# Amelie-Schreiber/ShapeMol

Measured on AMD Instinct MI355X. Metric: molecules/sec (1000-step DDPM sample, batch 256), higher is better.
Workload: dtype f32 (matrix operands split exactly into 3 x bf16 pieces = 24 bits, six piece products, fp32 accumulate); 1 GPU; BASELINE configs[1]: batch 256 MOSES-prior molecules (9-27 atoms) per GPU, 1000-step chain, fp32 results, k=8, synthetic shapes + hash-filled weights; besides the 5 warm-up steps an untimed 200-step chain runs first to reach the loaded clocks; batch_per_gpu=256, atoms_per_gpu=5541, total_atoms=5541, noise=device Philox, trajectories=kept in HBM, launch=hipGraph replay, parallelism=dp1 (whole batches per rank), ranks_seen=1

## Files before the change

shapemol_amd/csrc/shapemol_hip.hip:

```cpp
#include "../../include/shapemol_hip.h"
#include "sm_device.h"
#include "sm_edge.h"
#include "sm_edge_bf16.h"
#include "sm_edge16.h"
#include "sm_node.h"
#include "sm_node16.h"
#include "sm_edge_stream.h"
#include "sm_misc.h"
#include "sm_cfg.h"
#include "sm_guide_groups.h"
#include "sm_mesh.h"
#include <hip/hip_ext.h>

#include <algorithm>
#include <cmath>
#include <cstdio>
#include <cstring>
#include <map>
#include <string>
#include <type_traits>
#include <vector>

#include "sm_pack.h"
#include "sm_devmem.h"
// ... 82 lines not shown
    int num_cu = 256;
    CloudSet cs; MeshSet ms; DevList mem_cs, mem_ms;
    int2 *wg_table = nullptr; int64_t wg_table_cap = 0; DevList mem_wg;
    shapemol_sd_ctx *field_sd = nullptr; double field_lr = 0.0; int field_step = 0;
    float4 *m_within = nullptr; int *m_out = nullptr, *m_cnt = nullptr; int64_t m_cap = 0, m_cnt_cap = 0; DevList mem_mesh;
    int64_t m_flag_groups = 0;
    double cfg_w = 0.0, cfg_p = 0.0; int cfg_type = 0, cfg_has_bounds = 0; float cfg_lo[3] = {}, cfg_hi[3] = {};
    float *cfg_tr_pos_u = nullptr, *cfg_tr_v_u = nullptr;
    float *pred_pos_u = nullptr, *pred_v_u = nullptr;
    float *shape_zero = nullptr;
    float *cfg_stat = nullptr; double *cfg_part = nullptr; unsigned *cfg_hist = nullptr;
    CfgGroupSet cgs;
    int *cfg_mol_grp = nullptr; int2 *cfg_blk_tab = nullptr; double *cfg_gpart = nullptr; int64_t cfg_tab_stride = 0;
    int first_step = 0;
    int *pin_off = nullptr, *pin_atom = nullptr, *pin_nbr = nullptr; int64_t n_pins = 0; int pin_steps = 0, pin_k = 0; DevList mem_pins;
    bool prof_on = false;
    std::vector<ProfRec> prof;
    hipEvent_t cur_e0 = nullptr, cur_e1 = nullptr;
    hipGraphExec_t gexec = nullptr, gexec_u = nullptr;
    int64_t n_captures = 0;
    int64_t launch_rec[8] = {}, graph_rec[8] = {};
    int64_t node_rec[8] = {};
    int64_t x2h_out_rec[4] = {};
    struct GraphKey { int64_t N = 0, B = 0; Guide guide = Guide::None; int fold = 0, gfuse = 0;
                      int cfg = 0 ; double cfgv[9] = {};
                      int cfg_groups = 0;
                      uint64_t field_gen = 0; double field_lr = 0.0; int field_step = 0;
                      bool operator==(const GraphKey &o) const {
                          if (!(N == o.N && B == o.B && guide == o.guide && fold == o.fold && gfuse == o.gfuse && cfg == o.cfg &&
                                cfg_groups == o.cfg_groups && field_gen == o.field_gen && field_lr == o.field_lr &&
                                field_step == o.field_step)) return false;
                          for (int i = 0; i < 9; ++i) if (cfgv[i] != o.cfgv[i]) return false;
                          return true;
                      } } gkey{};
    hipStream_t gstream = nullptr; bool gstream_set = false;
    void drop_graphs() {
        if (!gexec && !gexec_u) return;
        if (!gstream_set || hipStreamSynchronize(gstream) != hipSuccess) hipDeviceSynchronize();
        if (gexec) { hipGraphExecDestroy(gexec); gexec = nullptr; }
        if (gexec_u) { hipGraphExecDestroy(gexec_u); gexec_u = nullptr; }
    }
    const float *P(size_t off) const { return d_img + off; }
};

namespace {

// ... 71 lines not shown
    if (N <= c->capN && B <= c->capB) return 0;
    HIPCHK(hipSetDevice(c->device));
    HIPCHK(hipDeviceSynchronize());
    c->drop_graphs();
    const int64_t capN = std::max<int64_t>(N, c->capN), capB = std::max<int64_t>(B, c->capB);
    c->ws.release();
    c->capN = c->capB = 0; c->lastN = c->lastB = 0; c->last_h = c->last_x = nullptr;
    if (workspace_alloc(c, capN, capB)) { c->ws.release(); return 1; }
    c->capN = capN; c->capB = capB;
    return 0;
}

}

#include "sm_guide_host.h"

namespace {

constexpr int kVnFoldBytes = kVnFoldCap * 3 * 4 + 32 * 8;

template <int H>
lg::In launch_in(const shapemol_ctx *c, int n_atoms) {
    constexpr bool chain16_fits = Chain16Lds<H>::BYTES <= 2 * EdgeImage16<H, H / 16>::TOTAL * 4;
    return {c->opt, {kVnFoldCap, kStreamTPR, CHAIN_COLS, kGraphCap, kLin6Chunk, chain16_fits}, c->KP, c->num_cu, H, n_atoms};
}

#define ATTR(bytes, ...) HIPCHK(hipFuncSetAttribute((const void *)__VA_ARGS__, hipFuncAttributeMaxDynamicSharedMemorySize, (int)(bytes)))
template <int H, int K>
int set_edge_attr_k() {
    constexpr int NT = H / 16;
    constexpr int vn_tail = vn_red_doubles(12, H / 8) * 8 + 12 * 96 * 4;
    constexpr int fold = K <= 16 ? kVnFoldBytes : 0;
    constexpr int x16 = 2 * EdgeImage16<H, NT>::TOTAL * 4 + fold, h16 = (EdgeImage16<H, NT>::TOTAL + EdgeImage16<H, 1>::TOTAL) * 4 + vn_tail;
    ATTR(x16, edge16_kernel<H, K, false>); ATTR(x16, edge16_kernel<H, K, false, true>);
    ATTR(x16, edge16_loop_kernel<H, K, false>); ATTR(x16, edge16_loop_kernel<H, K, false, true>);
    ATTR(h16, edge16_kernel<H, K, true>); ATTR(h16, edge16_kernel<H, K, true, true>);
    ATTR(h16, edge16_loop_kernel<H, K, true>); ATTR(h16, edge16_loop_kernel<H, K, true, true>);
    ATTR((StreamMap<H, false>::O_TAIL * 4 + kVnFoldBytes), edge_stream_kernel<H, K, false>);
    ATTR((StreamMap<H, true>::O_TAIL * 4 + (NT + kStreamProducers) * 64 * 2 * 8), edge_stream_kernel<H, K, true>);
    if constexpr (K <= 16) {
        constexpr int xph = EdgePhaseImage<H, NT>::TOTAL * 4, hph = (EdgePhaseImage<H, NT>::TOTAL + EdgePhaseImage<H, 1>::TOTAL) * 4 + vn_tail;
        ATTR(x16, x2h_chain16_kernel<H, K>); ATTR(x16, x2h_chain16_kernel<H, K, true>);
        ATTR((EdgeBlob<H, false>::TOTAL * 4), edge_attention_kernel<H, K, false>); ATTR((EdgeBlob<H, true>::TOTAL * 4), edge_attention_kernel<H, K, true>);
        ATTR(xph, edge_fused_kernel<H, K, false, false>); ATTR(xph, edge_fused_kernel<H, K, false, true>);
        ATTR(hph, edge_fused_kernel<H, K, true, false>); ATTR(hph, edge_fused_kernel<H, K, true, true>);
    }
    return 0;
// ... 321 lines not shown
        HIPCHK(c->mem_tab.alloc(&c->q_tab, rows * 5 * H * sizeof(float) + rows * (sizeof(int64_t) + sizeof(int)) + ((size_t)T + 1) * sizeof(int)));
        c->pre_tab = c->q_tab + rows * H;
        c->tab_v = reinterpret_cast<int64_t *>(c->pre_tab + rows * 4 * H);
        c->tab_mol_of = reinterpret_cast<int *>(c->tab_v + rows); c->tab_t_mol = c->tab_mol_of + rows; c->tab_flag = c->tab_t_mol + T;
    }
    c->tab_key = 0;
    LAUNCH("prep", SMK(prologue_tab_index_kernel, dim3((unsigned)((rows + 255) / 256)), dim3(256), 0, s, c->tab_v, c->tab_mol_of, c->tab_t_mol, c->tab_flag, T, C));
    const NodePrologueArgs pa = prologue_args<H>(c, c->tab_v, c->tab_mol_of, c->tab_t_mol, nullptr, c->etab, c->q_tab, c->pre_tab, (int)rows);
    if (launch_prologue<H>(c, s, pa, c->tab_flag)) return 1;
    c->tab_key = prologue_tab_key(c);
    return 0;
}

template <int H>
int run_score(shapemol_ctx *c, hipStream_t s, const ShapePrep &sp, const float *x_in, const int64_t *v_in, int64_t N, int64_t B,
              bool sampling, int t_first, float *out_pos, float *out_h, float *out_v, bool reuse_graph = false) {
    const shapemol_config &g = c->cfg;
    const int L = g.num_layers, hd = g.n_heads, C = g.num_classes, D = g.time_emb_dim, KP = c->KP;
    const int n = (int)N;
    AtomEmbArgs ae{c->P(c->dm.embw), c->P(c->dm.embb), v_in, c->mol_of, c->ttab, c->t_mol, sampling ? c->steps : nullptr,
                   c->steps + 1, c->bn_acc, c->h_a, n, H, C, D, t_first, L * kVnReplicas * 2 * hd + L};
    const int nlay = c->opt.stop_layer >= 0 ? std::min(c->opt.stop_layer, L) : L;
    const lg::In gi = launch_in<H>(c, n);
    const lg::StepForms sf = lg::step_forms(gi, sampling, c->n_pins > 0);
    if (sf.fused_prologue && c->opt.prologue_tab) {
        if (c->tab_key != prologue_tab_key(c)) return fail("run_score: the prologue tables are not built for this precision mode");
        PrologueTabArgs ta{c->etab, c->q_tab, c->pre_tab, c->tab_flag, v_in, c->mol_of, c->t_mol, ae.step_ptr, ae.step_cur, c->bn_acc,
                           sp.add0, c->h_a, c->q_x, c->pre0, c->status + ST_RANGE, n, C, g.num_timesteps, t_first, ae.bn_acc_len};
        LAUNCH("node_prologue", SMK(node_prologue_tab_kernel<H>, dim3((unsigned)((N * 16 + kProTabThreads - 1) / kProTabThreads)), dim3(kProTabThreads), 0, s, ta));
    } else if (sf.fused_prologue) {
        NodePrologueArgs pa = prologue_args<H>(c, v_in, c->mol_of, c->t_mol, sp.add0, c->h_a, c->q_x, c->pre0, n);
        pa.step_ptr = ae.step_ptr; pa.step_cur = ae.step_cur; pa.bn_acc = c->bn_acc; pa.bn_acc_len = ae.bn_acc_len; pa.t_first = t_first;
        if (nlay == 0) pa.n_lin_tiles = 0;
        pa.stamps = c->kstamp_sel == 5 ? c->kstamps : nullptr;
        if (launch_prologue<H>(c, s, pa)) return 1;
    } else {
        LAUNCH("embed", SMK(atom_embed_kernel, dim3((N * H + 255) / 256), dim3(256), 0, s, ae));
    }
    int64_t (&rec)[8] = c->launch_rec;
    std::fill(rec, rec + 8, 0);
    std::fill(c->node_rec, c->node_rec + 8, 0);
    std::fill(c->x2h_out_rec, c->x2h_out_rec + 4, 0);
    rec[0] = sampling; rec[1] = sf.graph_fused; rec[7] = c->num_cu;
    if (sf.stream && nlay > 0) { const lg::StreamGeom g = lg::stream_geom(gi); rec[5] = g.chunk; rec[6] = g.grid; }
    if (reuse_graph) {
    } else if (sf.graph_fused) {
        GraphArgs ga{x_in, c->mol_span, n, g.knn, KP, c->nbr, c->P(c->dm.ew.w1), c->P(c->dm.ew.b1), c->P(c->dm.ew.g), c->P(c->dm.ew.be),
                     c->P(c->dm.ew.w2), c->P(c->dm.ew.b2), c->ew, c->status + ST_SPAN, c->kstamp_sel == 4 ? c->kstamps : nullptr};
        const int apb = kGraphWaves * (KP >= 16 ? 1 : 16 / KP);
        DISPATCH_KP("graph", graph_kernel, (), dim3((n + apb - 1) / apb), dim3(kGraphWaves * 64), 0, s, ga);
    } else LAUNCH("knn", SMK(knn_kernel, dim3((N + 3) / 4), dim3(256), 0, s, x_in, c->mol_of, c->mol_off, n, g.knn, KP, c->nbr));
    if (sampling && c->n_pins > 0 && !reuse_graph)
        LAUNCH("knn", SMK(knn_pin_kernel, dim3(32), dim3(256), 0, s, c->pin_off, c->pin_steps, c->pin_atom, c->pin_nbr, c->pin_k, KP, c->steps + 1, n, c->nbr));
    EdgeWeightArgs ea{x_in, c->nbr, c->P(c->dm.ew.w1), c->P(c->dm.ew.b1), c->P(c->dm.ew.g), c->P(c->dm.ew.be),
                      c->P(c->dm.ew.w2), c->P(c->dm.ew.b2), c->ew, n * KP, KP};
    if (!sf.graph_fused && !reuse_graph) {
        const int tiles = (n * KP + 15) / 16;
        LAUNCH("edge_weight", SMK(edge_weight_kernel<H>, dim3((tiles + 3) / 4), dim3(256), 0, s, ea));
    }
    const float *cur_x = x_in;
    float *cur_h = c->h_a;
    constexpr int NT = H / 16;
    bool v_done = false;
    if (nlay > 0 && !sf.fused_prologue) {
        const DevLayer &D0 = c->dm.layer[0];
        if (launch_linear<H>(c, s, "node_pre", cur_h, c->P(D0.pre_x2h), c->P(D0.pre6_x2h), c->P(D0.pre16_x2h), sp.add0, 4 * H, c->pre0, 4 * H, 4 * NT, n,
                             c->kstamp_sel == 0 ? c->kstamps : nullptr)) return 1;
        if (launch_mlp2<H, 1>(c, s, "node_q", D0.q_x2h, cur_h, nullptr, NODE_LN_RELU, nullptr, c->q_x, H, H, n)) return 1;
    }
    double *stat_acc = c->bn_acc;
    if (c->bn_eval) {
        if (!c->bn_run) return fail("bn_eval = 1 needs the running statistics (shapemol_set_bn_running)");
        if (c->opt.vn_fuse == 1) return fail("bn_eval = 1 is not available with vn_fuse = 1 (coordinate update behind a grid barrier)");
// ... 319 lines not shown
            const double v[9] = {c->cfg_w, c->cfg_p, (double)c->cfg_has_bounds, c->cfg_lo[0], c->cfg_lo[1], c->cfg_lo[2], c->cfg_hi[0], c->cfg_hi[1], c->cfg_hi[2]};
            std::copy(v, v + 9, key.cfgv);
        }
        auto capture = [&](int n_steps, hipGraphExec_t *exec) -> int {
            hipGraph_t graph = nullptr;
            HIPCHK(hipStreamBeginCapture(s, hipStreamCaptureModeThreadLocal));
            int rc = 0;
            for (int i = 0; i < n_steps && !rc; ++i) rc = one_step();
            const hipError_t ce = hipStreamEndCapture(s, &graph);
            if (rc) { if (graph) hipGraphDestroy(graph); return 1; }
            if (ce != hipSuccess) return fail(std::string("hipStreamEndCapture: ") + hipGetErrorString(ce));
            const hipError_t ie = hipGraphInstantiate(exec, graph, nullptr, nullptr, 0);
            hipGraphDestroy(graph);
            if (ie != hipSuccess) { *exec = nullptr; return fail(std::string("hipGraphInstantiate: ") + hipGetErrorString(ie)); }
            ++c->n_captures;
            hipGraphUpload(*exec, s);
            return 0;
        };
        if (!c->gexec || !(key == c->gkey)) {
            c->drop_graphs();
            if (capture(1, &c->gexec)) return 1;
            c->gkey = key;
            std::copy(c->launch_rec, c->launch_rec + 8, c->graph_rec);
        }
        if (!c->gexec_u && capture(kGraphUnroll, &c->gexec_u)) return 1;
        int st = 0;
        c->gstream = s; c->gstream_set = true;
        std::copy(c->graph_rec, c->graph_rec + 8, c->launch_rec);
        for (; st + kGraphUnroll <= num_steps; st += kGraphUnroll) HIPCHK(hipGraphLaunch(c->gexec_u, s));
        for (; st < num_steps; ++st) HIPCHK(hipGraphLaunch(c->gexec, s));
    } else {
        for (int st = 0; st < num_steps; ++st) if (one_step()) return 1;
    }
    HIPCHK(hipMemcpyAsync(out_pos, c->x_state, N * 3 * sizeof(float), hipMemcpyDeviceToDevice, s));
    HIPCHK(hipMemcpyAsync(out_v, c->v_state, N * sizeof(int64_t), hipMemcpyDeviceToDevice, s));
    return 0;
}

int shapemol_log_sample_categorical(shapemol_ctx *c, const float *d_logits, const float *d_u, int64_t n_rows,
                                    int32_t n_classes, uint64_t seed, int64_t *out_index, void *stream) {
    if (!d_logits || !out_index || n_rows < 1 || n_classes < 1) return fail("shapemol_log_sample_categorical: bad argument");
    if (c) HIPCHK(hipSetDevice(c->device));
    hipStream_t s = (hipStream_t)stream;
    hipLaunchKernelGGL(gumbel_argmax_kernel, dim3((n_rows + 255) / 256), dim3(256), 0, s, d_logits, d_u, (int)n_rows, (int)n_classes, seed, out_index);
    HIPCHK(hipGetLastError());
    return 0;
}

int shapemol_set_option(shapemol_ctx *c, const char *name, int64_t value) {
    if (!c || !name) return fail("shapemol_set_option: null argument");
    const std::string k(name);
    if (k == "max_mol_atoms") {
        if (value < 0) return fail("max_mol_atoms must be >= 0");
        c->opt.max_mol_atoms = (int)std::min<int64_t>(value, 1 << 20);
        return 0;
    }
    if (k == "first_step") {
        if (value < 0 || value >= c->cfg.num_timesteps) return fail("first_step must be in [0, num_timesteps)");
        c->first_step = (int)value;
        return 0;
    }
    if (k == "stop_layer") c->opt.stop_layer = (int)value;
    else if (k == "edge_bf16") {
        if (value < 0 || value > 3) return fail("edge_bf16 must be 0 (fp32 MFMA), 1 (exactly split bf16, phase kernels), 2 (exactly split bf16, streaming kernels) or 3 (two-piece f16)");
        if (value != 3 && value != 2 && c->KP > 16) return fail("k > 16 runs on the streaming (edge_bf16 = 2) or the two-piece f16 (edge_bf16 = 3) edge kernels");
        if (value == 3 && c->hid_max > 6.0e4f) return fail("edge_bf16 = 3: the edge MLPs' LayerNorm outputs may exceed the fp16 range for these weights");
        c->opt.edge_bf16 = (int)value;
    }
    else if (k == "edge_tiles") { if (value < -1 || value > 1) return fail("edge_tiles must be -1 (automatic), 0 (sliced one-job launches) or 1 (looping launch)"); c->opt.edge_tiles = (int)value; }
    else if (k == "node_f16") c->opt.node_f16 = value != 0;
    else if (k == "feat_f16") {
        if (value && (c->opt.edge_bf16 != 3 || !c->opt.node_f16)) return fail("feat_f16 = 1 needs the f16 kernels (edge_bf16 = 3, node_f16 = 1)");
        c->opt.feat_f16 = value != 0;
    }
    else if (k == "lin_fuse") c->opt.lin_fuse = value != 0;
    else if (k == "stream_whole_rounds") c->opt.stream_whole_rounds = value != 0;
    else if (k == "x2h_chain") c->opt.x2h_chain = value != 0;
    else if (k == "graph_fuse") c->opt.graph_fuse = value != 0;
    else if (k == "bn_eval") c->bn_eval = value != 0;
    else if (k == "ddpm_fold") c->opt.ddpm_fold = value != 0;
    else if (k == "vn_fold") c->opt.vn_fold = value != 0;
    else if (k == "prologue_tab") c->opt.prologue_tab = value != 0;
    else if (k == "lin_bf16") c->opt.lin_bf16 = (int)value;
    else if (k == "chain_bf16") c->opt.chain_bf16 = (int)value;
    else if (k == "vn_fuse") c->opt.vn_fuse = (int)value;
    else if (k == "node_levels") c->opt.node_levels = value != 0;
    else if (k == "x2h_out_fuse") { if (value < 0 || value > 2) return fail("x2h_out_fuse must be 0 (node_out6_kernel), 1 (x2h tail inside its boundary) or 2 (x2h tail always)"); c->opt.x2h_out_fuse = (int)value; }
    else if (k == "stream_chunk") { if (value < 0 || value > 4096) return fail("stream_chunk must be 0 (automatic) .. 4096"); c->opt.stream_chunk_opt = (int)value; }
    else if (k == "after_order") { if (value < 0 || value > 2) return fail("after_order must be 0 (follow-up jobs first), 1 (interleaved) or 2 (linear jobs first)"); c->opt.after_order = (int)value; }
    else if (k == "after_waves") { if (value < 1 || value > 16) return fail("after_waves must be 1..16"); c->opt.after_waves = (int)value; }
    else if (k == "after_lin_wgs") { if (value < 0 || value > 4096) return fail("after_lin_wgs must be 0 (automatic) .. 4096"); c->opt.after_lin_wgs = (int)value; }
    else if (k == "lin_waves") { if (value < 1 || value > 16) return fail("lin_waves must be 1..16"); c->opt.lin_waves = (int)value; }
    else if (k == "stamps") c->stamp_on = (int)value;
    else if (k == "kstamp_sel") c->kstamp_sel = (int)value;
    else if (k == "edge_waves") { if (value < 0 || value > 12) return fail("edge_waves must be 0 (automatic) .. 12"); c->opt.edge_threads = (int)value * 64; }
    else return fail("unknown option " + k);
    hipSetDevice(c->device);
    c->drop_graphs();
    return 0;
}

int64_t shapemol_debug_read(shapemol_ctx *c, const char *name, void *dst, size_t max_bytes) {
    if (!c || !name || !dst) { fail("shapemol_debug_read: null argument"); return -1; }
    const std::string k(name);
    const shapemol_config &g = c->cfg;
    const int64_t N = c->lastN;
    const void *src = nullptr; size_t bytes = 0;
    int64_t dims[8] = {N, c->lastB, c->KP, g.hidden_dim, g.n_heads, g.num_layers, c->capN, c->capB};
    if (k == "dims") { if (max_bytes < sizeof(dims)) return -1; std::memcpy(dst, dims, sizeof(dims)); return sizeof(dims); }
    if (k == "captures") { if (max_bytes < 8) return -1; std::memcpy(dst, &c->n_captures, 8); return 8; }
    if (k == "launch") { if (max_bytes < sizeof(c->launch_rec)) return -1; std::memcpy(dst, c->launch_rec, sizeof(c->launch_rec)); return sizeof(c->launch_rec); }
    if (k == "launch_x2h_out") { if (max_bytes < sizeof(c->x2h_out_rec)) return -1; std::memcpy(dst, c->x2h_out_rec, sizeof(c->x2h_out_rec)); return sizeof(c->x2h_out_rec); }
    if (k == "launch_node") { if (max_bytes < sizeof(c->node_rec)) return -1; std::memcpy(dst, c->node_rec, sizeof(c->node_rec)); return sizeof(c->node_rec); }
    if (k == "nbr") { src = c->nbr; bytes = N * c->KP * 4; }
    else if (k == "ew") { src = c->ew; bytes = N * c->KP * 4; }
    else if (k == "h") { src = c->last_h; bytes = N * g.hidden_dim * 4; }
    else if (k == "x") { src = c->last_x; bytes = N * 3 * 4; }
    else if (k == "h0") { src = c->h_a; bytes = N * g.hidden_dim * 4; }
    else if (k == "q_x") { src = c->q_x; bytes = N * g.hidden_dim * 4; }
    else if (k == "pre0") { src = c->pre0; bytes = N * 4 * g.hidden_dim * 4; }
    else if (k == "add0") { src = c->prep[0].add0; bytes = (size_t)c->lastB * 4 * g.hidden_dim * 4; }
    else if (k == "pre") { src = c->preAB; bytes = N * 8 * g.hidden_dim * 4; }
    else if (k == "q") { src = c->q_h; bytes = N * g.hidden_dim * 4; }
    else if (k == "att") { src = c->att; bytes = N * g.hidden_dim * 4; }
    else if (k == "o3") { src = c->o3; bytes = N * 48 * 4; }
    else if (k == "stamps") { src = c->stamps; bytes = 2048 * 8; }
    else if (k == "kstamps") { src = c->kstamps; bytes = (size_t)8 * 16 * 4096 * 8; }
    else if (k == "vn_err") { src = c->status + ST_VN_BARRIER; bytes = 4; }
    else if (k == "mesh_group_flags") { src = c->m_cnt ? c->m_cnt + 4 * c->m_cnt_cap : nullptr; bytes = (size_t)c->m_flag_groups * 4; }
    else if (k == "cfg_stat") { src = c->cfg_stat; bytes = 2 * 4; }
    else if (k == "cfg_group_stat") { src = c->cgs.last_groups > 0 ? c->cgs.stat : nullptr; bytes = (size_t)c->cgs.last_groups * 2 * 4; }
    else if (k == "bnstat") { src = c->bn_acc; bytes = (size_t)g.num_layers * kVnReplicas * 2 * g.n_heads * 8; }
    else { fail("shapemol_debug_read: unknown buffer " + k); return -1; }
    if (!src || bytes > max_bytes) { fail("shapemol_debug_read: buffer unavailable or destination too small"); return -1; }
    if (hipSetDevice(c->device) != hipSuccess || hipDeviceSynchronize() != hipSuccess ||
        hipMemcpy(dst, src, bytes, hipMemcpyDeviceToHost) != hipSuccess) { fail("shapemol_debug_read: copy failed"); return -1; }
    return (int64_t)bytes;
}

int shapemol_debug_cfg_stats(shapemol_ctx *c, const float *d_pos_cond, const float *d_pos_uncond, const float *d_v_cond, const float *d_v_uncond,
                             const int64_t *d_batch, int64_t N, int64_t B, void *stream) {
    const std::string me = "shapemol_debug_cfg_stats: ";
    if (!c || !d_pos_cond || !d_pos_uncond || !d_v_cond || !d_v_uncond || !d_batch) return fail(me + "null argument");
    if (N < 1 || B < 1 || B > N || N > (1 << 27) || N * c->cfg.num_classes >= (int64_t)1 << 31) return fail(me + "n_atoms / n_mols out of range");
    if (chain_guide(c) != Guide::Cfg) return fail(me + "no classifier-free guidance setting is installed (or another guidance takes precedence)");
    if (c->cgs.groups > 0 && c->cgs.mols != B)
        return fail(me + "n_mols = " + std::to_string(B) + " but the classifier-free guidance groups cover " + std::to_string(c->cgs.mols) + " molecules");
    HIPCHK(hipSetDevice(c->device));
// ... 167 lines not shown
```

shapemol_amd/csrc/sm_launch.h:

```cpp
#pragma once
#include <algorithm>

namespace lg {

struct Options {
    int stop_layer = -1, edge_threads = 0 , lin_waves = 16, edge_bf16 = 2, lin_bf16 = 1, chain_bf16 = 1, vn_fuse = 2;
    int vn_fold = 1;
    int max_mol_atoms = 0;
    int stream_whole_rounds = 0;
    int lin_fuse = 0;
    int ddpm_fold = 1;
    int graph_fuse = 1;
    int x2h_chain = 1;
    int node_levels = 1;
    int x2h_out_fuse = 1;
    int stream_chunk_opt = 0;
    int after_order = 2;
    int after_waves = 16;
    int after_lin_wgs = 0;
    int node_f16 = 0;
    int feat_f16 = 0;
    int edge_tiles = -1;
    int prologue_tab = 1;
};

struct KernelConsts { int vn_fold_cap, stream_tpr, chain_cols, graph_cap, lin6_chunk; bool chain16_fits; };

struct In { Options o; KernelConsts k; int KP, num_cu, H, n_atoms; };

inline int cdiv(int a, int b) { return (a + b - 1) / b; }

struct Jobs { int apj, jobs; bool half; };
inline Jobs tile_jobs(int KP, int n_atoms) {
    const int apj = KP >= 16 ? 1 : 16 / KP;
    return {apj, KP > 16 ? 2 * n_atoms : cdiv(n_atoms, apj), KP > 16};
}

enum class Form { One, Loop, Sliced, Strided };
struct EdgeGeom { Form form; int apj, jobs, waves, grid, chunk, slice, atoms_per_wg; };

inline int edge_waves(const In &in, int jobs) {
    return in.o.edge_threads > 0 ? in.o.edge_threads / 64 : std::max(4, std::min(12, cdiv(jobs, in.num_cu)));
}
inline EdgeGeom one_job_geom(const In &in, int waves) {
    const Jobs j = tile_jobs(in.KP, in.n_atoms);
    const int grid = std::max(1, std::min(in.num_cu, cdiv(j.jobs, waves)));
    return {j.jobs <= grid * waves ? Form::One : Form::Strided, j.apj, j.jobs, waves, grid, waves, grid * waves, j.half ? 0 : waves * j.apj};
}

// ... 60 lines not shown
    return {n_ct, waves, ogroups, tpg, cdiv(n_ct, tpg)};
}

constexpr int kAfterChunk = 6;
struct NodeLevelsGeom { int n_ct, n_pairs, lw, bw, n_fjobs, n_ljobs, tpg, lin_chunk; };
inline NodeLevelsGeom node_levels_geom(const In &in, int n_follow, int lin_tiles) {
    NodeLevelsGeom g{};
    g.n_ct = cdiv(in.n_atoms, 16); g.n_pairs = cdiv(g.n_ct, in.k.chain_cols);
    g.lw = in.o.after_waves; g.bw = std::max(g.lw, in.H / 16);
    const int per_cu = g.bw <= 8 ? 2 : 1;
    const int slots = in.num_cu * per_cu;
    g.n_fjobs = n_follow * g.n_pairs;
    g.tpg = 1;
    if (lin_tiles > 0) {
        const int ogroups = cdiv(lin_tiles, g.lw);
        const int lin_wgs = in.o.after_lin_wgs > 0 ? in.o.after_lin_wgs : std::max(slots - g.n_fjobs, slots / 2);
        g.tpg = std::max(1, cdiv(g.n_ct, std::max(1, lin_wgs / ogroups)));
        g.n_ljobs = ogroups * cdiv(g.n_ct, g.tpg);
    }
    g.lin_chunk = std::min(g.tpg, per_cu == 2 ? kAfterChunk : in.k.lin6_chunk);
    return g;
}

struct StepForms {
    bool fused_prologue;
    bool graph_fused;
    bool fold;
    bool f16, stream, phases;
    bool half_tiles;
    bool lin_fused;
    bool levels;
    bool out_fused;
    bool xc_fused;
};
inline StepForms step_forms(const In &in, bool sampling, bool pins) {
    const Options &o = in.o;
    const int KP = in.KP, m = o.max_mol_atoms;
    StepForms f{};
    f.fused_prologue = o.chain_bf16 && o.lin_bf16;
    f.graph_fused = sampling && o.graph_fuse && m > 0 && m <= in.k.graph_cap && KP <= 32 && !pins;
    f.f16 = o.edge_bf16 == 3; f.stream = o.edge_bf16 == 2; f.phases = o.edge_bf16 && KP <= 16;
    f.half_tiles = (f.f16 || f.stream) && KP > 16;
    f.lin_fused = o.chain_bf16 && o.lin_bf16 && o.node_f16 && o.lin_fuse;
    f.levels = o.node_levels && o.chain_bf16 && o.lin_bf16 && !o.node_f16 && !f.lin_fused;
    const StreamGeom sg = stream_geom(in);
    const EdgeGeom e16 = edge16_geom(in), xc = x2h_chain_geom(in);
    f.xc_fused = f.f16 && o.x2h_chain && KP <= 16 && o.chain_bf16 && o.node_f16 && !o.lin_fuse && o.edge_threads == 0 &&
                 xc.form == Form::One && xc.waves <= 12 && xc.atoms_per_wg <= in.k.chain_cols * 16 && in.k.chain16_fits;
    f.out_fused = f.stream && o.x2h_out_fuse && f.levels && KP <= 16 && (o.x2h_out_fuse == 2 || sg.atoms_per_wg <= 3 * in.k.chain_cols * 16);
    const int own = f.stream ? sg.atoms_per_wg : std::max(e16.atoms_per_wg, xc.atoms_per_wg);
    f.fold = sampling && o.vn_fold && (f.f16 || f.stream) && KP <= 16 && o.vn_fuse == 2 && m > 0 && (f.stream || o.edge_threads == 0) &&
             own + 2 * (m - 1) <= in.k.vn_fold_cap;
    return f;
}

}
```

shapemol_amd/csrc/sm_misc.h:

```cpp
#pragma once
#include "sm_device.h"
#include "sm_cfg.h"
#include "sm_vn.h"

enum StatusFlag { ST_VN_BARRIER = 0, ST_BATCH = 1, ST_ATOM_TYPE = 2, ST_TIME = 3, ST_RANGE = 4, ST_SPAN = 5, ST_MESH = 6 };

__global__ void mol_index_kernel(const int64_t *batch, int n, int n_mols, int *mol_of, int *mol_off, int *status) {
    const int i = blockIdx.x * blockDim.x + threadIdx.x;
    if (i >= n) return;
    const int64_t braw = batch[i], praw = i == 0 ? -1 : batch[i - 1];
    if (braw < 0 || braw >= n_mols || braw < praw) status[ST_BATCH] = 1;
    const int b = (int)min(max(braw, (int64_t)0), (int64_t)n_mols - 1);
    const int prev = (int)min(max(praw, (int64_t)-1), (int64_t)n_mols - 1);
    mol_of[i] = b;
    for (int m = prev + 1; m <= b; ++m) mol_off[m] = i;
    if (i == n - 1)
        for (int m = b + 1; m <= n_mols; ++m) mol_off[m] = n;
}

__global__ void mol_span_kernel(const int *mol_of, const int *mol_off, int n, int2 *span) {
    const int i = blockIdx.x * blockDim.x + threadIdx.x;
    if (i < n) span[i] = int2{mol_off[mol_of[i]], mol_off[mol_of[i] + 1]};
}

__global__ void t_convert_kernel(const int64_t *t, int n_mols, int n_timesteps, int *t_mol, int *status) {
    const int i = blockIdx.x * blockDim.x + threadIdx.x;
// ... 187 lines not shown
    float y = a.b[f] + w[min(max((int)a.v[i], 0), a.C - 1)];
    const float *te = a.ttab + (size_t)t * a.D;
    for (int k = 0; k < a.D; ++k) y += w[a.C + k] * te[k];
    a.h[idx] = y;
}

struct PrologueTabArgs {
    const float *etab, *q_tab, *pre_tab;
    const int *tab_flag;
    const int64_t *v;
    const int *mol_of;
    const int *t_mol;
    const int *step_ptr;
    int *step_cur;
    double *bn_acc;
    const float *add_mol;
    float *h_out, *q_out, *pre_out;
    int *range_flag;
    int n_atoms, C, T, t_first, bn_acc_len;
};

constexpr int kProTabThreads = 256;

template <int H>
__global__ void __launch_bounds__(kProTabThreads)
node_prologue_tab_kernel(PrologueTabArgs a) {
    constexpr int R = H / 64;
    static_assert(H % 64 == 0 || H == 32, "16 lanes x 16 bytes cover a row in whole passes");
    const int gid = blockIdx.x * kProTabThreads + threadIdx.x;
    const int step = a.step_ptr ? *a.step_ptr : 0;
    if (gid == 0) {
        if (a.step_ptr) *a.step_cur = step;
        if (*a.tab_flag) *a.range_flag = 1;
    }
    for (int i = gid; i < a.bn_acc_len; i += gridDim.x * kProTabThreads) a.bn_acc[i] = 0.0;
    const int atom = gid >> 4, ln = gid & 15;
    if (atom >= a.n_atoms) return;
    const int mol = a.mol_of[atom];
    const int t = min(max(a.step_ptr ? a.t_first - step : a.t_mol[mol], 0), a.T - 1);
    const int vi = min(max((int)a.v[atom], 0), a.C - 1);
    const size_t row = (size_t)t * a.C + vi;
    if constexpr (H == 32) {
        const int f = 4 * (ln & 7);
        const float *src = (ln < 8 ? a.etab : a.q_tab) + row * H + f;
        const float4 hq = ldg4(src);
        const float4 p0 = ldg4(a.pre_tab + row * 4 * H + 4 * ln), p1 = ldg4(a.pre_tab + row * 4 * H + 64 + 4 * ln);
        const float4 m0 = ldg4(a.add_mol + (size_t)mol * 4 * H + 4 * ln), m1 = ldg4(a.add_mol + (size_t)mol * 4 * H + 64 + 4 * ln);
        stg4((ln < 8 ? a.h_out : a.q_out) + (size_t)atom * H + f, hq);
        stg4(a.pre_out + (size_t)atom * 4 * H + 4 * ln, float4{p0.x + m0.x, p0.y + m0.y, p0.z + m0.z, p0.w + m0.w});
        stg4(a.pre_out + (size_t)atom * 4 * H + 64 + 4 * ln, float4{p1.x + m1.x, p1.y + m1.y, p1.z + m1.z, p1.w + m1.w});
    } else {
        float4 h[R], q[R], p[4 * R], m[4 * R];
#pragma unroll
        for (int r = 0; r < R; ++r) {
            h[r] = ldg4(a.etab + row * H + 64 * r + 4 * ln);
            q[r] = ldg4(a.q_tab + row * H + 64 * r + 4 * ln);
        }
#pragma unroll
        for (int r = 0; r < 4 * R; ++r) {
            p[r] = ldg4(a.pre_tab + row * 4 * H + 64 * r + 4 * ln);
            m[r] = ldg4(a.add_mol + (size_t)mol * 4 * H + 64 * r + 4 * ln);
        }
#pragma unroll
        for (int r = 0; r < R; ++r) {
            stg4(a.h_out + (size_t)atom * H + 64 * r + 4 * ln, h[r]);
            stg4(a.q_out + (size_t)atom * H + 64 * r + 4 * ln, q[r]);
        }
#pragma unroll
        for (int r = 0; r < 4 * R; ++r)
            stg4(a.pre_out + (size_t)atom * 4 * H + 64 * r + 4 * ln, float4{p[r].x + m[r].x, p[r].y + m[r].y, p[r].z + m[r].z, p[r].w + m[r].w});
    }
}

__global__ void prologue_tab_index_kernel(int64_t *v, int *mol_of, int *t_mol, int *flag, int T, int C) {
    const int i = blockIdx.x * blockDim.x + threadIdx.x;
    if (i == 0) *flag = 0;
    if (i < T) t_mol[i] = i;
    if (i < T * C) { v[i] = i % C; mol_of[i] = i / C; }
}

SM_DEV float dist2_rounded(float dx, float dy, float dz) {
#pragma clang fp contract(off)
    const float a = dx * dx, b = dy * dy, c = dz * dz;
    return (a + b) + c;
}

__global__ void knn_kernel(const float *x, const int *mol_of, const int *mol_off, int n_atoms, int k,
                           int kp, int *nbr) {
    const int lane = threadIdx.x & 63;
    const int i = blockIdx.x * (blockDim.x >> 6) + (threadIdx.x >> 6);
    if (i >= n_atoms) return;
    const int m = mol_of[i], s = mol_off[m], cnt = mol_off[m + 1] - s;
    const float xi = x[i * 3], yi = x[i * 3 + 1], zi = x[i * 3 + 2];
    const int deg = min(k, cnt - 1);
// ... 141 lines not shown
    red[threadIdx.x][0] = o[0]; red[threadIdx.x][1] = o[1]; red[threadIdx.x][2] = o[2];
    __syncthreads();
    if (ok && c < 3) {
        float res = 0.f;
        for (int h = 0; h < heads; ++h) res += red[la * heads + h][c];
        const float att = vn_rows_sum(a.o3 + (size_t)i * 48, c);
        a.x_out[i * 3 + c] = a.x[i * 3 + c] + (att / heads + res / heads);
    }
}

constexpr int kGraphCap = 128;
constexpr int kGraphWaves = 8;
struct GraphArgs {
    const float *x;
    const int2 *mol_span;
    int n_atoms, k, kp;
    int *nbr;
    const float *w1, *b1, *g, *be, *w2, *b2;
    float *ew;
    int *span_flag;
    unsigned long long *stamps;
};
template <int H, int KP>
__global__ void __launch_bounds__(kGraphWaves * 64)
graph_kernel(GraphArgs a) {
    constexpr int NT = H / 16;
    constexpr int APW = KP >= 16 ? 1 : 16 / KP;
    constexpr int LPA = 64 / APW;
    constexpr int NQ = kGraphCap / LPA;
    constexpr int TPW = KP > 16 ? KP / 16 : 1;
    __shared__ float w1s[H * 20];
    __shared__ unsigned long long dkey[kGraphWaves][APW][kGraphCap];
    __shared__ float xs[kGraphWaves][APW][kGraphCap][3];
    __shared__ int row[kGraphWaves][APW * KP];
    __shared__ __attribute__((aligned(16))) float prm[4][H];
    const int lane = threadIdx.x & 63, wave = threadIdx.x >> 6;
    const int n = lane & 15, g = lane >> 4;
    const int sub = lane / LPA, l = lane % LPA;
    const int i_raw = (blockIdx.x * kGraphWaves + wave) * APW + sub;
    const bool valid = i_raw < a.n_atoms;
    const int i = valid ? i_raw : a.n_atoms - 1;
    SM_TICK(a.stamps, 0);
    const int2 span = a.mol_span[i];
    for (int idx = threadIdx.x; idx < H * 20; idx += kGraphWaves * 64) w1s[idx] = a.w1[idx];
    for (int idx = threadIdx.x; idx < 4 * H; idx += kGraphWaves * 64) {
        const int which = idx / H, f = idx % H;
        prm[which][f] = (which == 0 ? a.b1 : which == 1 ? a.g : which == 2 ? a.be : a.w2)[f];
    }
    const float b2 = a.b2[0];
    const float *x = a.x;
    const int s = span.x, cnt = min(span.y - span.x, kGraphCap), self = i - s;
    if (span.y - span.x > kGraphCap && l == 0) *a.span_flag = 1;
    const float xi = x[i * 3], yi = x[i * 3 + 1], zi = x[i * 3 + 2];
    float dc[NQ];
#pragma unroll
    for (int q = 0; q < NQ; ++q) {
        const int c = l + LPA * q;
        dc[q] = 0.f;
        if (c < cnt) {
            const int j = s + c;
            const float xj = x[j * 3], yj = x[j * 3 + 1], zj = x[j * 3 + 2];
            const float dx = xj - xi, dy = yj - yi, dz = zj - zi;
// ... 15 lines not shown
#pragma unroll
    for (int q = 0; q < NQ; ++q) kc[q] = ((unsigned long long)__builtin_bit_cast(unsigned, dc[q]) << 32) | (unsigned)(l + LPA * q);
    for (int o = 0; o < cnt; ++o) {
        const unsigned long long k_o = dkey[wave][sub][o];
#pragma unroll
        for (int q = 0; q < NQ; ++q) {
            if (q >= nq_w) break;
            rank[q] += k_o < kc[q];
        }
    }
#pragma unroll
    for (int q = 0; q < NQ; ++q) {
        const int c = l + LPA * q;
        if (c < cnt && c != self && rank[q] < a.k) row[wave][sub * KP + rank[q]] = s + c;
    }
    __builtin_amdgcn_fence(__ATOMIC_RELEASE, "wavefront");
    __builtin_amdgcn_wave_barrier();
    __builtin_amdgcn_fence(__ATOMIC_ACQUIRE, "wavefront");
    SM_TICK(a.stamps, 3);
    if (valid)
        for (int sl = l; sl < KP; sl += LPA) a.nbr[(size_t)i * KP + sl] = row[wave][sub * KP + sl];
    float cen[5];
    rbf_centres(g, cen);
    const int atom0 = (blockIdx.x * kGraphWaves + wave) * APW;
#pragma unroll
    for (int tt = 0; tt < TPW; ++tt) {
        const int slot = tt * 16 + n;
        const int asub = slot / KP;
        const int ia_raw = atom0 + asub;
        const bool in_range = ia_raw < a.n_atoms;
        const int ia = in_range ? ia_raw : a.n_atoms - 1;
        const int jraw = in_range ? row[wave][slot] : -1;
        const bool ok = in_range && jraw >= 0;
        const int s_a = __shfl(s, asub * LPA), self_a = __shfl(self, asub * LPA);
        const int cj = ok ? jraw - s_a : self_a;
        const float *pa = xs[wave][asub][self_a], *pj = xs[wave][asub][cj];
        const float r0 = pa[0] - pj[0], r1 = pa[1] - pj[1], r2 = pa[2] - pj[2];
        float rb[5];
        rbf_dlayout(sqrtf(r0 * r0 + r1 * r1 + r2 * r2), cen, rb);
        float hid[NT * 4];
#pragma unroll
        for (int t = 0; t < NT; ++t) {
            const float4 b = ldg4(prm[0] + 16 * t + 4 * g);
            f32x4 acc = {b.x, b.y, b.z, b.w};
#pragma unroll
            for (int s5 = 0; s5 < 5; ++s5) acc = mfma16(w1s[(16 * t + n) * 20 + 4 * s5 + g], rb[s5], acc);
            hid[4 * t] = acc[0]; hid[4 * t + 1] = acc[1]; hid[4 * t + 2] = acc[2]; hid[4 * t + 3] = acc[3];
        }
        SM_TICK(a.stamps, 4);
        ln_relu_dlayout<NT>(hid, prm[1], prm[2], g);
        SM_TICK(a.stamps, 5);
        float p = 0.f;
#pragma unroll
        for (int t = 0; t < NT; ++t) {
            const float4 w = ldg4(prm[3] + 16 * t + 4 * g);
            p += w.x * hid[4 * t] + w.y * hid[4 * t + 1] + w.z * hid[4 * t + 2] + w.w * hid[4 * t + 3];
        }
        p = sum_groups(p) + b2;
        if (g == 0 && in_range) a.ew[(size_t)ia * KP + slot % KP] = ok ? 1.0f / (1.0f + expf(-p)) : 0.f;
    }
    SM_STAMP(a.stamps, 6);
}

struct ChainParams {
    unsigned long long seed;
    const float *eps, *u;
    float *tr_pos; int64_t *tr_v; float *tr_v0; float *tr_vt; float *tr_pos_cond; float *tr_v_cond;
    float *tr_pos_uncond; float *tr_v_uncond;
    const double *guide_draws;
    int step_base;
};
__global__ void set_chain_params_kernel(ChainParams *dst, ChainParams v, int *step_counter) { *dst = v; *step_counter = v.step_base; }

struct DdpmFold {
    const float *pd;
    const double *acc;
    const float *bn_g, *bn_b;
    const float *xsum;
    const float *x_old;
    float *pred_out;
    int heads, enable;
};
struct DdpmArgs {
    const float *pred_pos;
// ... 310 lines not shown
```

Measured before the change: 397.3 molecules/s.

## Fuse graph kernel and prologue table gather into one step-head launch

Adds a step_head_kernel whose blocks are split between kNN/edge-weight graph jobs and prologue table gather jobs, replacing two separate launches per denoising step when graph fusion and prologue tables are active. The aim is to remove one kernel boundary per step and let the light gather work overlap the graph work on idle CUs. The gather path now uses the graph kernel's block size and a smaller register batch (PW=2), which may change its memory-level parallelism. Block ordering is configurable and defaults to graph jobs first.

```diff
diff --git a/shapemol_amd/csrc/shapemol_hip.hip b/shapemol_amd/csrc/shapemol_hip.hip
--- a/shapemol_amd/csrc/shapemol_hip.hip
+++ b/shapemol_amd/csrc/shapemol_hip.hip
@@ -128,6 +128,7 @@
     int64_t launch_rec[8] = {}, graph_rec[8] = {};
     int64_t node_rec[8] = {};
     int64_t x2h_out_rec[4] = {};
+    int64_t head_rec[4] = {}, graph_head_rec[4] = {};
     struct GraphKey { int64_t N = 0, B = 0; Guide guide = Guide::None; int fold = 0, gfuse = 0;
                       int cfg = 0 ; double cfgv[9] = {};
                       int cfg_groups = 0;
@@ -245,7 +246,7 @@
 template <int H>
 lg::In launch_in(const shapemol_ctx *c, int n_atoms) {
     constexpr bool chain16_fits = Chain16Lds<H>::BYTES <= 2 * EdgeImage16<H, H / 16>::TOTAL * 4;
-    return {c->opt, {kVnFoldCap, kStreamTPR, CHAIN_COLS, kGraphCap, kLin6Chunk, chain16_fits}, c->KP, c->num_cu, H, n_atoms};
+    return {c->opt, {kVnFoldCap, kStreamTPR, CHAIN_COLS, kGraphCap, kLin6Chunk, chain16_fits, kGraphWaves}, c->KP, c->num_cu, H, n_atoms};
 }
 
 #define ATTR(bytes, ...) HIPCHK(hipFuncSetAttribute((const void *)__VA_ARGS__, hipFuncAttributeMaxDynamicSharedMemorySize, (int)(bytes)))
@@ -613,12 +614,26 @@
                    c->steps + 1, c->bn_acc, c->h_a, n, H, C, D, t_first, L * kVnReplicas * 2 * hd + L};
     const int nlay = c->opt.stop_layer >= 0 ? std::min(c->opt.stop_layer, L) : L;
     const lg::In gi = launch_in<H>(c, n);
-    const lg::StepForms sf = lg::step_forms(gi, sampling, c->n_pins > 0);
+    const lg::StepForms sf = lg::step_forms(gi, sampling, c->n_pins > 0, reuse_graph);
+    const GraphArgs ga{x_in, c->mol_span, n, g.knn, KP, c->nbr, c->P(c->dm.ew.w1), c->P(c->dm.ew.b1), c->P(c->dm.ew.g), c->P(c->dm.ew.be),
+                       c->P(c->dm.ew.w2), c->P(c->dm.ew.b2), c->ew, c->status + ST_SPAN, c->kstamp_sel == 4 ? c->kstamps : nullptr};
+    const int graph_apb = kGraphWaves * (KP >= 16 ? 1 : 16 / KP);
+    int64_t (&hrec)[4] = c->head_rec;
+    std::fill(hrec, hrec + 4, 0);
+    hrec[3] = c->opt.head_order;
+    if (sf.graph_fused && !reuse_graph) hrec[1] = (n + graph_apb - 1) / graph_apb;
     if (sf.fused_prologue && c->opt.prologue_tab) {
         if (c->tab_key != prologue_tab_key(c)) return fail("run_score: the prologue tables are not built for this precision mode");
         PrologueTabArgs ta{c->etab, c->q_tab, c->pre_tab, c->tab_flag, v_in, c->mol_of, c->t_mol, ae.step_ptr, ae.step_cur, c->bn_acc,
                            sp.add0, c->h_a, c->q_x, c->pre0, c->status + ST_RANGE, n, C, g.num_timesteps, t_first, ae.bn_acc_len};
-        LAUNCH("node_prologue", SMK(node_prologue_tab_kernel<H>, dim3((unsigned)((N * 16 + kProTabThreads - 1) / kProTabThreads)), dim3(kProTabThreads), 0, s, ta));
+        if (sf.head_fused) {
+            const lg::HeadGeom hg = lg::head_geom(gi);
+            hrec[0] = 1; hrec[1] = hg.n_graph; hrec[2] = hg.n_gather;
+            DISPATCH_KP("graph", step_head_kernel, (), dim3((unsigned)(hg.n_graph + hg.n_gather)), dim3(kGraphWaves * 64), 0, s, ga, ta, hg);
+        } else {
+            hrec[2] = (N * 16 + kProTabThreads - 1) / kProTabThreads;
+            LAUNCH("node_prologue", SMK(node_prologue_tab_kernel<H>, dim3((unsigned)hrec[2]), dim3(kProTabThreads), 0, s, ta));
+        }
     } else if (sf.fused_prologue) {
         NodePrologueArgs pa = prologue_args<H>(c, v_in, c->mol_of, c->t_mol, sp.add0, c->h_a, c->q_x, c->pre0, n);
         pa.step_ptr = ae.step_ptr; pa.step_cur = ae.step_cur; pa.bn_acc = c->bn_acc; pa.bn_acc_len = ae.bn_acc_len; pa.t_first = t_first;
@@ -636,10 +651,7 @@
     if (sf.stream && nlay > 0) { const lg::StreamGeom g = lg::stream_geom(gi); rec[5] = g.chunk; rec[6] = g.grid; }
     if (reuse_graph) {
     } else if (sf.graph_fused) {
-        GraphArgs ga{x_in, c->mol_span, n, g.knn, KP, c->nbr, c->P(c->dm.ew.w1), c->P(c->dm.ew.b1), c->P(c->dm.ew.g), c->P(c->dm.ew.be),
-                     c->P(c->dm.ew.w2), c->P(c->dm.ew.b2), c->ew, c->status + ST_SPAN, c->kstamp_sel == 4 ? c->kstamps : nullptr};
-        const int apb = kGraphWaves * (KP >= 16 ? 1 : 16 / KP);
-        DISPATCH_KP("graph", graph_kernel, (), dim3((n + apb - 1) / apb), dim3(kGraphWaves * 64), 0, s, ga);
+        if (!sf.head_fused) DISPATCH_KP("graph", graph_kernel, (), dim3((n + graph_apb - 1) / graph_apb), dim3(kGraphWaves * 64), 0, s, ga);
     } else LAUNCH("knn", SMK(knn_kernel, dim3((N + 3) / 4), dim3(256), 0, s, x_in, c->mol_of, c->mol_off, n, g.knn, KP, c->nbr));
     if (sampling && c->n_pins > 0 && !reuse_graph)
         LAUNCH("knn", SMK(knn_pin_kernel, dim3(32), dim3(256), 0, s, c->pin_off, c->pin_steps, c->pin_atom, c->pin_nbr, c->pin_k, KP, c->steps + 1, n, c->nbr));
@@ -1005,11 +1017,13 @@
             if (capture(1, &c->gexec)) return 1;
             c->gkey = key;
             std::copy(c->launch_rec, c->launch_rec + 8, c->graph_rec);
+            std::copy(c->head_rec, c->head_rec + 4, c->graph_head_rec);
         }
         if (!c->gexec_u && capture(kGraphUnroll, &c->gexec_u)) return 1;
         int st = 0;
         c->gstream = s; c->gstream_set = true;
         std::copy(c->graph_rec, c->graph_rec + 8, c->launch_rec);
+        std::copy(c->graph_head_rec, c->graph_head_rec + 4, c->head_rec);
         for (; st + kGraphUnroll <= num_steps; st += kGraphUnroll) HIPCHK(hipGraphLaunch(c->gexec_u, s));
         for (; st < num_steps; ++st) HIPCHK(hipGraphLaunch(c->gexec, s));
     } else {
@@ -1041,6 +1055,14 @@
     if (k == "first_step") {
         if (value < 0 || value >= c->cfg.num_timesteps) return fail("first_step must be in [0, num_timesteps)");
         c->first_step = (int)value;
+        return 0;
+    }
+    if (k == "debug_tab_flag") {
+        if (!c->tab_flag) return fail("debug_tab_flag: the prologue tables are not built yet");
+        const int v = value != 0;
+        HIPCHK(hipSetDevice(c->device));
+        HIPCHK(hipDeviceSynchronize());
+        HIPCHK(hipMemcpy(c->tab_flag, &v, sizeof(int), hipMemcpyHostToDevice));
         return 0;
     }
     if (k == "stop_layer") c->opt.stop_layer = (int)value;
@@ -1064,6 +1086,8 @@
     else if (k == "ddpm_fold") c->opt.ddpm_fold = value != 0;
     else if (k == "vn_fold") c->opt.vn_fold = value != 0;
     else if (k == "prologue_tab") c->opt.prologue_tab = value != 0;
+    else if (k == "head_fuse") c->opt.head_fuse = value != 0;
+    else if (k == "head_order") { if (value < 0 || value > 2) return fail("head_order must be 0 (graph jobs first), 1 (gather jobs first) or 2 (interleaved)"); c->opt.head_order = (int)value; }
     else if (k == "lin_bf16") c->opt.lin_bf16 = (int)value;
     else if (k == "chain_bf16") c->opt.chain_bf16 = (int)value;
     else if (k == "vn_fuse") c->opt.vn_fuse = (int)value;
@@ -1095,6 +1119,7 @@
     if (k == "launch") { if (max_bytes < sizeof(c->launch_rec)) return -1; std::memcpy(dst, c->launch_rec, sizeof(c->launch_rec)); return sizeof(c->launch_rec); }
     if (k == "launch_x2h_out") { if (max_bytes < sizeof(c->x2h_out_rec)) return -1; std::memcpy(dst, c->x2h_out_rec, sizeof(c->x2h_out_rec)); return sizeof(c->x2h_out_rec); }
     if (k == "launch_node") { if (max_bytes < sizeof(c->node_rec)) return -1; std::memcpy(dst, c->node_rec, sizeof(c->node_rec)); return sizeof(c->node_rec); }
+    if (k == "launch_head") { if (max_bytes < sizeof(c->head_rec)) return -1; std::memcpy(dst, c->head_rec, sizeof(c->head_rec)); return sizeof(c->head_rec); }
     if (k == "nbr") { src = c->nbr; bytes = N * c->KP * 4; }
     else if (k == "ew") { src = c->ew; bytes = N * c->KP * 4; }
     else if (k == "h") { src = c->last_h; bytes = N * g.hidden_dim * 4; }
@@ -1107,6 +1132,7 @@
     else if (k == "q") { src = c->q_h; bytes = N * g.hidden_dim * 4; }
     else if (k == "att") { src = c->att; bytes = N * g.hidden_dim * 4; }
     else if (k == "o3") { src = c->o3; bytes = N * 48 * 4; }
+    else if (k == "steps") { src = c->steps; bytes = 2 * 4; }
     else if (k == "stamps") { src = c->stamps; bytes = 2048 * 8; }
     else if (k == "kstamps") { src = c->kstamps; bytes = (size_t)8 * 16 * 4096 * 8; }
     else if (k == "vn_err") { src = c->status + ST_VN_BARRIER; bytes = 4; }
diff --git a/shapemol_amd/csrc/sm_launch.h b/shapemol_amd/csrc/sm_launch.h
--- a/shapemol_amd/csrc/sm_launch.h
+++ b/shapemol_amd/csrc/sm_launch.h
@@ -22,9 +22,11 @@
     int feat_f16 = 0;
     int edge_tiles = -1;
     int prologue_tab = 1;
+    int head_fuse = 1;
+    int head_order = 0;
 };
 
-struct KernelConsts { int vn_fold_cap, stream_tpr, chain_cols, graph_cap, lin6_chunk; bool chain16_fits; };
+struct KernelConsts { int vn_fold_cap, stream_tpr, chain_cols, graph_cap, lin6_chunk; bool chain16_fits; int graph_waves = 8; };
 
 struct In { Options o; KernelConsts k; int KP, num_cu, H, n_atoms; };
 
@@ -131,6 +133,20 @@
     return g;
 }
 
+struct HeadGeom { int n_graph, n_gather, order, n_tri; };
+struct HeadJob { bool gather; int blk; };
+inline HeadGeom head_geom(const In &in) {
+    const int apb = in.k.graph_waves * tile_jobs(in.KP, in.n_atoms).apj, gpb = in.k.graph_waves * 64 / 16;
+    const int n_graph = cdiv(in.n_atoms, apb), n_gather = cdiv(in.n_atoms, gpb);
+    return {n_graph, n_gather, in.o.head_order, in.o.head_order == 2 ? std::min(n_graph / 2, n_gather) : 0};
+}
+constexpr HeadJob head_job(const HeadGeom &g, int b) {
+    if (g.order == 1) return b < g.n_gather ? HeadJob{true, b} : HeadJob{false, b - g.n_gather};
+    if (b < 3 * g.n_tri) return b % 3 == 2 ? HeadJob{true, b / 3} : HeadJob{false, b / 3 * 2 + b % 3};
+    const int rest = b - 3 * g.n_tri, graph_left = g.n_graph - 2 * g.n_tri;
+    return rest < graph_left ? HeadJob{false, 2 * g.n_tri + rest} : HeadJob{true, g.n_tri + rest - graph_left};
+}
+
 struct StepForms {
     bool fused_prologue;
     bool graph_fused;
@@ -141,13 +157,15 @@
     bool levels;
     bool out_fused;
     bool xc_fused;
+    bool head_fused;
 };
-inline StepForms step_forms(const In &in, bool sampling, bool pins) {
+inline StepForms step_forms(const In &in, bool sampling, bool pins, bool reuse_graph = false) {
     const Options &o = in.o;
     const int KP = in.KP, m = o.max_mol_atoms;
     StepForms f{};
     f.fused_prologue = o.chain_bf16 && o.lin_bf16;
     f.graph_fused = sampling && o.graph_fuse && m > 0 && m <= in.k.graph_cap && KP <= 32 && !pins;
+    f.head_fused = f.fused_prologue && o.prologue_tab && f.graph_fused && o.head_fuse && !reuse_graph;
     f.f16 = o.edge_bf16 == 3; f.stream = o.edge_bf16 == 2; f.phases = o.edge_bf16 && KP <= 16;
     f.half_tiles = (f.f16 || f.stream) && KP > 16;
     f.lin_fused = o.chain_bf16 && o.lin_bf16 && o.node_f16 && o.lin_fuse;
diff --git a/shapemol_amd/csrc/sm_misc.h b/shapemol_amd/csrc/sm_misc.h
--- a/shapemol_amd/csrc/sm_misc.h
+++ b/shapemol_amd/csrc/sm_misc.h
@@ -2,6 +2,7 @@
 #include "sm_device.h"
 #include "sm_cfg.h"
 #include "sm_vn.h"
+#include "sm_launch.h"
 
 enum StatusFlag { ST_VN_BARRIER = 0, ST_BATCH = 1, ST_ATOM_TYPE = 2, ST_TIME = 3, ST_RANGE = 4, ST_SPAN = 5, ST_MESH = 6 };
 
@@ -235,18 +236,17 @@
 
 constexpr int kProTabThreads = 256;
 
-template <int H>
-__global__ void __launch_bounds__(kProTabThreads)
-node_prologue_tab_kernel(PrologueTabArgs a) {
+template <int THREADS, int H, int PW = 4 * (H / 64)>
+SM_DEV void prologue_tab_job(const PrologueTabArgs &a, int blk, int n_blk) {
     constexpr int R = H / 64;
     static_assert(H % 64 == 0 || H == 32, "16 lanes x 16 bytes cover a row in whole passes");
-    const int gid = blockIdx.x * kProTabThreads + threadIdx.x;
+    const int gid = blk * THREADS + threadIdx.x;
     const int step = a.step_ptr ? *a.step_ptr : 0;
     if (gid == 0) {
         if (a.step_ptr) *a.step_cur = step;
         if (*a.tab_flag) *a.range_flag = 1;
     }
-    for (int i = gid; i < a.bn_acc_len; i += gridDim.x * kProTabThreads) a.bn_acc[i] = 0.0;
+    for (int i = gid; i < a.bn_acc_len; i += n_blk * THREADS) a.bn_acc[i] = 0.0;
     const int atom = gid >> 4, ln = gid & 15;
     if (atom >= a.n_atoms) return;
     const int mol = a.mol_of[atom];
@@ -263,26 +263,41 @@
         stg4(a.pre_out + (size_t)atom * 4 * H + 4 * ln, float4{p0.x + m0.x, p0.y + m0.y, p0.z + m0.z, p0.w + m0.w});
         stg4(a.pre_out + (size_t)atom * 4 * H + 64 + 4 * ln, float4{p1.x + m1.x, p1.y + m1.y, p1.z + m1.z, p1.w + m1.w});
     } else {
-        float4 h[R], q[R], p[4 * R], m[4 * R];
+        constexpr int NP = 4 * R;
+        static_assert(PW >= 1 && NP % PW == 0, "whole passes over the pre_tab row");
+        float4 h[R], q[R], p[PW], m[PW];
+        auto store_hq = [&]() {
+#pragma unroll
+            for (int r = 0; r < R; ++r) {
+                stg4(a.h_out + (size_t)atom * H + 64 * r + 4 * ln, h[r]);
+                stg4(a.q_out + (size_t)atom * H + 64 * r + 4 * ln, q[r]);
+            }
+        };
 #pragma unroll
         for (int r = 0; r < R; ++r) {
             h[r] = ldg4(a.etab + row * H + 64 * r + 4 * ln);
             q[r] = ldg4(a.q_tab + row * H + 64 * r + 4 * ln);
         }
-#pragma unroll
-        for (int r = 0; r < 4 * R; ++r) {
-            p[r] = ldg4(a.pre_tab + row * 4 * H + 64 * r + 4 * ln);
-            m[r] = ldg4(a.add_mol + (size_t)mol * 4 * H + 64 * r + 4 * ln);
-        }
-#pragma unroll
-        for (int r = 0; r < R; ++r) {
-            stg4(a.h_out + (size_t)atom * H + 64 * r + 4 * ln, h[r]);
-            stg4(a.q_out + (size_t)atom * H + 64 * r + 4 * ln, q[r]);
-        }
-#pragma unroll
-        for (int r = 0; r < 4 * R; ++r)
-            stg4(a.pre_out + (size_t)atom * 4 * H + 64 * r + 4 * ln, float4{p[r].x + m[r].x, p[r].y + m[r].y, p[r].z + m[r].z, p[r].w + m[r].w});
-    }
+        if constexpr (PW < NP) store_hq();
+#pragma unroll
+        for (int r0 = 0; r0 < NP; r0 += PW) {
+#pragma unroll
+            for (int r = 0; r < PW; ++r) {
+                p[r] = ldg4(a.pre_tab + row * 4 * H + 64 * (r0 + r) + 4 * ln);
+                m[r] = ldg4(a.add_mol + (size_t)mol * 4 * H + 64 * (r0 + r) + 4 * ln);
+            }
+            if constexpr (PW == NP) store_hq();
+#pragma unroll
+            for (int r = 0; r < PW; ++r)
+                stg4(a.pre_out + (size_t)atom * 4 * H + 64 * (r0 + r) + 4 * ln, float4{p[r].x + m[r].x, p[r].y + m[r].y, p[r].z + m[r].z, p[r].w + m[r].w});
+        }
+    }
+}
+
+template <int H>
+__global__ void __launch_bounds__(kProTabThreads)
+node_prologue_tab_kernel(PrologueTabArgs a) {
+    prologue_tab_job<kProTabThreads, H>(a, blockIdx.x, gridDim.x);
 }
 
 __global__ void prologue_tab_index_kernel(int64_t *v, int *mol_of, int *t_mol, int *flag, int T, int C) {
@@ -470,8 +485,7 @@
     unsigned long long *stamps;
 };
 template <int H, int KP>
-__global__ void __launch_bounds__(kGraphWaves * 64)
-graph_kernel(GraphArgs a) {
+SM_DEV void graph_job(const GraphArgs &a, unsigned blk) {
     constexpr int NT = H / 16;
     constexpr int APW = KP >= 16 ? 1 : 16 / KP;
     constexpr int LPA = 64 / APW;
@@ -485,7 +499,7 @@
     const int lane = threadIdx.x & 63, wave = threadIdx.x >> 6;
     const int n = lane & 15, g = lane >> 4;
     const int sub = lane / LPA, l = lane % LPA;
-    const int i_raw = (blockIdx.x * kGraphWaves + wave) * APW + sub;
+    const int i_raw = (blk * kGraphWaves + wave) * APW + sub;
     const bool valid = i_raw < a.n_atoms;
     const int i = valid ? i_raw : a.n_atoms - 1;
     SM_TICK(a.stamps, 0);
@@ -547,9 +561,10 @@
         for (int sl = l; sl < KP; sl += LPA) a.nbr[(size_t)i * KP + sl] = row[wave][sub * KP + sl];
     float cen[5];
     rbf_centres(g, cen);
-    const int atom0 = (blockIdx.x * kGraphWaves + wave) * APW;
+    const int atom0 = (blk * kGraphWaves + wave) * APW;
 #pragma unroll
     for (int tt = 0; tt < TPW; ++tt) {
+        if constexpr (TPW > 1) asm volatile("" ::: "memory");
         const int slot = tt * 16 + n;
         const int asub = slot / KP;
         const int ia_raw = atom0 + asub;
@@ -585,6 +600,20 @@
         if (g == 0 && in_range) a.ew[(size_t)ia * KP + slot % KP] = ok ? 1.0f / (1.0f + expf(-p)) : 0.f;
     }
     SM_STAMP(a.stamps, 6);
+}
+
+template <int H, int KP>
+__global__ void __launch_bounds__(kGraphWaves * 64)
+graph_kernel(GraphArgs a) {
+    graph_job<H, KP>(a, blockIdx.x);
+}
+
+template <int H, int KP>
+__global__ void __launch_bounds__(kGraphWaves * 64)
+step_head_kernel(GraphArgs ga, PrologueTabArgs ta, lg::HeadGeom hg) {
+    const lg::HeadJob job = lg::head_job(hg, (int)blockIdx.x);
+    if (job.gather) prologue_tab_job<kGraphWaves * 64, H, 2>(ta, job.blk, hg.n_gather);
+    else graph_job<H, KP>(ga, (unsigned)job.blk);
 }
 
 struct ChainParams {
```

Result: no change. 399.8 molecules/s (median of 6 runs) (+0.6%).
